# pacellie/raytracer_challenge

Measured on AMD Instinct MI355X. Metric: Mrays/s (unique rays: primary+shadow+reflection+refraction) at 1920x1080 depth-5, higher is better.
Workload: dtype f64

## Files before the change

### raytracer_challenge_amd/csrc/device_scene.h

```cpp
#pragma once
#include <stddef.h>
#include <stdint.h>

enum { OP_PRIM = 0, OP_GROUP = 1, OP_MESH = 2, OP_BVH = 3, OP_QUIRK = 4, OP_QGRID = 5, OP_CSG = 6, OP_CSG_END = 7 };

struct DOp {
  int32_t op, a, b, c;
  int32_t g;
  int32_t pad[3];
};

#define RTC_KOPS 12
#define RTC_KPLANES 6
struct DPlaneK {
  double row[4];
  int32_t prim;
  int32_t gcond;
  int32_t pad[2];
  double n[3];
};

struct DBvhNode {
  float lo0[3], hi0[3];
  float lo1[3], hi1[3];
// ... 165 lines not shown

struct DStats {
  unsigned long long rays_primary, rays_shadow, rays_reflect, rays_refract, rays_container;
  unsigned long long accel_nodes, group_tests, tri_tests, analytic_tests;
  unsigned long long knodes;
  unsigned long long kplanes;
  unsigned long long light_cells;
  unsigned long long kgroups;
  unsigned long long diag[64];
  unsigned long long nan_ts;
  unsigned long long guard;
  unsigned long long guard_claim;
  long long guard_info[8];
  unsigned long long wf_overflow;
};
#define RTC_STATS_LAUNCH_BYTES offsetof(DStats, nan_ts)

#define RTC_MAX_FUEL 16

#if defined(__HIPCC__) || defined(RTC_EMU)
#define RTC_HD __host__ __device__
#else
#define RTC_HD
#endif
static inline RTC_HD unsigned long long rtc_mix64(unsigned long long x) {
  x ^= x >> 33; x *= 0xff51afd7ed558ccdull; x ^= x >> 33; x *= 0xc4ceb9fe1a85ec53ull; x ^= x >> 33;
  return x;
}
static inline RTC_HD unsigned long long rtc_hit_hash_base(unsigned long long t_bits, int32_t prim, int32_t push) {
  return rtc_mix64(t_bits) ^ ((((unsigned long long)(uint32_t)prim << 32) | (unsigned long long)(uint32_t)push) * 0x9E3779B97F4A7C15ull);
}
static inline RTC_HD unsigned long long rtc_hit_hash(unsigned long long base, int depth, int kind) {
  return rtc_mix64(base ^ ((unsigned long long)(((unsigned)depth << 8) | (unsigned)kind) + 1ull) * 0xD6E8FEB86659FD93ull);
}

static inline RTC_HD unsigned long long rtc_splitmix64(unsigned long long z) {
  z = (z ^ (z >> 30)) * 0xbf58476d1ce4e5b9ull; z = (z ^ (z >> 27)) * 0x94d049bb133111ebull;
  return z ^ (z >> 31);
}
static inline RTC_HD unsigned long long rtc_area_hash(int light, double x, double y, double z) {
  unsigned long long bx, by, bz;
  __builtin_memcpy(&bx, &x, 8); __builtin_memcpy(&by, &y, 8); __builtin_memcpy(&bz, &z, 8);
  return rtc_splitmix64(rtc_splitmix64(rtc_splitmix64(rtc_splitmix64((unsigned long long)(uint32_t)light) ^ bx) ^ by) ^ bz);
}
static inline RTC_HD double rtc_area_jitter(unsigned long long h, unsigned j) {
  return (double)(rtc_splitmix64(h ^ (unsigned long long)j) >> 11) * 0x1.0p-53;
}
#define RTC_ALIGHT 16
#define RTC_SLIGHT 22

#define RTC_WF_SHADE_COUNT 32
#define RTC_WF_OVERFLOW 63
#define RTC_WF_CHUNK_NEXT 64
#define RTC_WF_COUNTS (64 + 32 * 8 * (RTC_MAX_FUEL + 2))
#ifndef RTC_WF_CHUNK
#define RTC_WF_CHUNK 64u
#endif
#define RTC_SR_PLAIN 0x40000000
#define RTC_WF_MISS (-2)
struct DWave {
  double* rq[2];
  double* h_t;
  int32_t* h_prim;
  double* h_n12;
  double* sr;
  int32_t* sr_mat;
  int32_t* sr_node;
  double* contrib;
  int32_t* child;
  uint32_t* counts;
  uint32_t cap;
  uint32_t pad;
  unsigned long long* dig;
};
static inline uint64_t dwave_bytes(uint64_t cap, int levels) {
  return cap * (uint64_t)(7 + 7 + 1 + 2 + 9 + 3 * levels) * sizeof(double) + (cap * (uint64_t)(1 + 1 + 1 + 2 * levels) + RTC_WF_COUNTS) * sizeof(int32_t);
}
static inline void dwave_carve(DWave* W, void* mem, uint64_t cap, int levels) {
  double* d = (double*)mem;
  W->rq[0] = d; d += 7 * cap;
  W->rq[1] = d; d += 7 * cap;
  W->h_t = d; d += cap;
  W->h_n12 = d; d += 2 * cap;
  W->sr = d; d += 9 * cap;
  W->contrib = d; d += 3 * (uint64_t)levels * cap;
  int32_t* q = (int32_t*)d;
  W->h_prim = q; q += cap;
  W->sr_mat = q; q += cap;
  W->sr_node = q; q += cap;
  W->child = q; q += 2 * (uint64_t)levels * cap;
  W->counts = (uint32_t*)q;
  W->cap = (uint32_t)cap;
  W->pad = 0;
  W->dig = nullptr;
}
#ifndef RTC_BVH_STACK
#define RTC_BVH_STACK 64
#endif
```

### raytracer_challenge_amd/csrc/rtc_background.hip

```cpp
#include "rtc_device.hpp"

#ifdef RTC_BG_BUILD

template <>
void rtc_launch_trace_bg_build<RTC_BG_BUILD>(const RtcFrame& F, const DBackground& bg, unsigned grid, int fuel, double* rgb) {
  constexpr RtcVariant R = RTC_BG_BUILDS[RTC_BG_BUILD];
  DSceneBg S;
  static_cast<DScene&>(S) = F.S;
  S.bg = bg;
  if (F.count)
    hipLaunchKernelGGL((rtc_trace_kernel<true, R.feat, R.kops, 0, false, R.area, R.uv, R.spot, true>), dim3(grid), dim3(RTC_BLOCK), rtc_stack_bytes(F.S), F.stream, S, F.cam, F.pm, fuel,
                       rgb, F.hit_t, F.hit_prim, F.hit_k, F.stats);
  else
    hipLaunchKernelGGL((rtc_trace_kernel<false, R.feat, R.kops, 0, false, R.area, R.uv, R.spot, true>), dim3(grid), dim3(RTC_BLOCK), rtc_stack_bytes(F.S), F.stream, S, F.cam, F.pm, fuel,
                       rgb, F.hit_t, F.hit_prim, F.hit_k, F.stats);
}

#else

uint64_t rtc_wavefront_work(const DCamera& cam, const DPixelMap& pm);

template <bool UV>
__global__ void __launch_bounds__(256) wf_background(DScene S, DCamera cam, DPixelMap pm, DWave W, int level, unsigned n0, DBackground bg) {
  const WorkMap wm = make_workmap(pm, cam);
  const unsigned count = wf_count(W, level, n0);
  const size_t cap = W.cap;
  int32_t* ch = W.child + (size_t)level * 2 * cap;
  double* cb = W.contrib + (size_t)level * 3 * cap;
  const double* rq = W.rq[level & 1];
  for (unsigned long long i = (unsigned long long)blockIdx.x * blockDim.x + threadIdx.x; i < count; i += (unsigned long long)gridDim.x * blockDim.x) {
    double dx, dy, dz, weight = 1.0;
    if (level == 0) {
      uint64_t q = 0;
      if (!work_to_slot(wm, i, q)) continue;
      if (ch[i] != RTC_WF_MISS) continue;
      const Ray r = slot_ray(pm, cam, q);
      dx = r.dx; dy = r.dy; dz = r.dz;
    } else {
      if (ch[i] != RTC_WF_MISS) continue;
      dx = rq[3 * cap + i]; dy = rq[4 * cap + i]; dz = rq[5 * cap + i];
      weight = rq[6 * cap + i];
    }
    double r, g, b;
    background_color<UV>(S, bg, dx, dy, dz, r, g, b);
    cb[i] = weight * r; cb[cap + i] = weight * g; cb[2 * cap + i] = weight * b;
    ch[i] = -1;
  }
}

void rtc_launch_wf_background(const DScene& S, const DCamera& cam, const DPixelMap& pm, const DWave& W, int level, unsigned n0, const DBackground& bg, unsigned blocks,
                              hipStream_t stream) {
  const unsigned long long most = level == 0 ? n0 : W.cap;
  const dim3 grid((unsigned)std::max<unsigned long long>(1ull, std::min<unsigned long long>((most + 255ull) / 256ull, (unsigned long long)std::max(1u, blocks)))), block(256);
  if (S.has_uv) hipLaunchKernelGGL(wf_background<true>, grid, block, 0, stream, S, cam, pm, W, level, n0, bg);
  else hipLaunchKernelGGL(wf_background<false>, grid, block, 0, stream, S, cam, pm, W, level, n0, bg);
}

template <bool UV>
__global__ void __launch_bounds__(256) rtc_background_colors_kernel(DScene S, DBackground bg, const double* __restrict__ dirs, unsigned long long n, double* __restrict__ rgb) {
  for (unsigned long long i = (unsigned long long)blockIdx.x * blockDim.x + threadIdx.x; i < n; i += (unsigned long long)gridDim.x * blockDim.x) {
    double r, g, b;
    background_color<UV>(S, bg, dirs[3 * i], dirs[3 * i + 1], dirs[3 * i + 2], r, g, b);
    rgb[3 * i] = r; rgb[3 * i + 1] = g; rgb[3 * i + 2] = b;
  }
}
void rtc_launch_background_colors(const DScene& S, const DBackground& bg, const double* dirs, unsigned long long n, double* rgb, hipStream_t stream) {
  if (n == 0) return;
  const dim3 grid((unsigned)std::min<unsigned long long>((n + 255ull) / 256ull, 8192ull)), block(256);
  if (S.has_uv) hipLaunchKernelGGL(rtc_background_colors_kernel<true>, grid, block, 0, stream, S, bg, dirs, n, rgb);
  else hipLaunchKernelGGL(rtc_background_colors_kernel<false>, grid, block, 0, stream, S, bg, dirs, n, rgb);
}

void rtc_launch_trace_bg(const DScene& S, const DBackground& bg, const DCamera& cam, const DPixelMap& pm, int fuel, double* rgb, double* hit_t, int* hit_prim, int* hit_k,
                         DStats* stats, bool count, hipStream_t stream) {
  if (pm.n == 0) return;
  const unsigned grid = (unsigned)((rtc_wavefront_work(cam, pm) + RTC_BLOCK - 1) / RTC_BLOCK);
  const RtcFrame F = {S, cam, pm, hit_t, hit_prim, hit_k, stats, stream, count};
  switch (rtc_pick_bg_build(S.has_area != 0, S.has_uv != 0, S.has_spot != 0)) {
    case 0: return rtc_launch_trace_bg_build<0>(F, bg, grid, fuel, rgb);
    case 1: return rtc_launch_trace_bg_build<1>(F, bg, grid, fuel, rgb);
    case 2: return rtc_launch_trace_bg_build<2>(F, bg, grid, fuel, rgb);
    case 3: return rtc_launch_trace_bg_build<3>(F, bg, grid, fuel, rgb);
    case 4: return rtc_launch_trace_bg_build<4>(F, bg, grid, fuel, rgb);
// ... 7 lines not shown
```

### raytracer_challenge_amd/csrc/rtc_device.hpp

```cpp
#pragma once

#include <hip/hip_runtime.h>
#include <stdint.h>

#include <algorithm>
#include <type_traits>

#include "background_point.h"
#include "device_scene.h"
#include "spot_factor.h"

#define EPS 0.00001
#ifndef RTC_BLOCK
#define RTC_BLOCK 64
#endif
#ifndef RTC_WAVES_PER_SIMD
#define RTC_WAVES_PER_SIMD 1
#endif
#ifdef RTC_TRAVERSE_NOINLINE
#define TRAVERSE_INLINE __noinline__
#else
#define TRAVERSE_INLINE __forceinline__
#endif
#ifndef RTC_LANE_ID
// ... 1484 lines not shown
            Pending& p = pend[np++];
            p.ox = st.ux; p.oy = st.uy; p.oz = st.uz; p.dx = spawn.tdx; p.dy = spawn.tdy; p.dz = spawn.tdz;
            p.weight = spawn.wt; p.fuel = fuel - 1; p.kind = 2;
          }
          if (spawn.refl) {
            ray.ox = st.px; ray.oy = st.py; ray.oz = st.pz; ray.dx = st.rx; ray.dy = st.ry; ray.dz = st.rz;
            weight = spawn.wr; fuel = fuel - 1; kind = 1;
            continue;
          }
          if (spawn.refr) {
            ray.ox = st.ux; ray.oy = st.uy; ray.oz = st.uz; ray.dx = spawn.tdx; ray.dy = spawn.tdy; ray.dz = spawn.tdz;
            weight = spawn.wt; fuel = fuel - 1; kind = 2;
            continue;
          }
        }
      } else if constexpr (BG) {
        double br, bgr, bb;
        background_color<UV>(S, S.bg, ray.dx, ray.dy, ray.dz, br, bgr, bb);
        acc_r += weight * br; acc_g += weight * bgr; acc_b += weight * bb;
      }
      DIAG_REGION(5);
      if (np == 0) {
        rgb[3 * q + 0] = acc_r;
        rgb[3 * q + 1] = acc_g;
        rgb[3 * q + 2] = acc_b;
        if (COUNT && pm.digest) pm.digest[q] = dg;
        break;
      }
      const Pending& p = pend[--np];
      ray.ox = p.ox; ray.oy = p.oy; ray.oz = p.oz; ray.dx = p.dx; ray.dy = p.dy; ray.dz = p.dz;
      weight = p.weight; fuel = p.fuel; kind = p.kind;
    }
  }

#ifdef RTC_DIAG
  atomicAdd(&s_diag[14], __builtin_amdgcn_s_memtime() - diag_k0);
  atomicAdd(&s_diag[15], 1ull);
  __syncthreads();
  if (threadIdx.x < 64 && s_diag[threadIdx.x]) atomicAdd(&stats->diag[threadIdx.x], s_diag[threadIdx.x]);
#endif
  if (C.nan_ts) atomicAdd(&stats->nan_ts, (unsigned long long)C.nan_ts);
  if (COUNT) {
    atomicAdd(&stats->rays_primary, (unsigned long long)n_primary);
    atomicAdd(&stats->rays_shadow, (unsigned long long)n_shadow);
    atomicAdd(&stats->rays_reflect, (unsigned long long)n_reflect);
    atomicAdd(&stats->rays_refract, (unsigned long long)n_refract);
    atomicAdd(&stats->rays_container, (unsigned long long)n_container);
    publish_counters(stats, C);
  }
}

namespace {

__device__ __forceinline__ unsigned wf_count(const DWave& W, int level, unsigned n0) {
  if (level == 0) return n0;
  unsigned c = W.counts[level];
  return c < W.cap ? c : W.cap;
}
__device__ __forceinline__ Ray wf_load_ray(const DWave& W, int level, unsigned i, double& weight) {
  const double* q = W.rq[level & 1];
  const size_t cap = W.cap;
  Ray r;
  r.ox = q[i]; r.oy = q[cap + i]; r.oz = q[2 * cap + i]; r.dx = q[3 * cap + i]; r.dy = q[4 * cap + i]; r.dz = q[5 * cap + i];
  weight = q[6 * cap + i];
  return r;
}

struct RecView {
  double ex, ey, ez, weight;
};
__device__ __forceinline__ RecView shade_rec_view(const DCamera& cam, const DPixelMap& pm, const DWave& W, const WorkMap& wm, int level, int node) {
  if (level == 0) {
    uint64_t q = 0;
    (void)work_to_slot(wm, (unsigned)node, q);
    const Ray pr = slot_ray(pm, cam, q);
    return {-pr.dx, -pr.dy, -pr.dz, 1.0};
  }
  const double* rq = W.rq[level & 1];
  const size_t cap = W.cap;
  return {-rq[3 * cap + node], -rq[4 * cap + node], -rq[5 * cap + node], rq[6 * cap + node]};
}
__device__ __forceinline__ const double* shade_rec_material(const DScene& S, const DWave& W, unsigned s, double& cr, double& cg, double& cb) {
  const double* r = W.sr;
  const size_t cap = W.cap;
  const int mrow = W.sr_mat[s];
  const double* M = S.mat + 8 * (mrow & (RTC_SR_PLAIN - 1));
  if (mrow & RTC_SR_PLAIN) { cr = M[4]; cg = M[5]; cb = M[6]; }
  else { cr = r[6 * cap + s]; cg = r[7 * cap + s]; cb = r[8 * cap + s]; }
  return M;
}
__device__ __forceinline__ const double* shade_rec_material_row(const DScene& S, const DWave& W, unsigned s, int mrow, double& cr, double& cg, double& cb) {
  const double* r = W.sr;
  const size_t cap = W.cap;
  const double* M = S.mat + 8 * (mrow & (RTC_SR_PLAIN - 1));
  if (mrow & RTC_SR_PLAIN) { cr = M[4]; cg = M[5]; cb = M[6]; }
  else { cr = r[6 * cap + s]; cg = r[7 * cap + s]; cb = r[8 * cap + s]; }
  return M;
}

}

template <int FEAT, bool KOPS, bool LDSC>
__device__ __forceinline__ void wf_trace_ray(const DScene& S, const DCamera& cam, const DPixelMap& pm, const DWave& W, const WorkMap& wm, int level, unsigned i,
                                             double* __restrict__ hit_t, int* __restrict__ hit_prim, int* __restrict__ hit_k, int* stack, int stride, Counters& C,
                                             unsigned& n_rays, unsigned& n_container, int fuel_left, const LdsScene& L, bool digest = false) {
  const size_t cap = W.cap;
  int32_t* ch = W.child + (size_t)level * 2 * cap;
  Ray ray;
  uint64_t q = 0;
  if (level == 0) {
    if (!work_to_slot(wm, i, q)) { W.h_prim[i] = -1; return; }
// ... 87 lines not shown
    if (RTC_PROBE & 8) RTC_LAUNDER(qx);
    const ShadowRay sh = shadow_ray(qx, py, pz, LG[3], LG[4], LG[5]);
    phong_add(LG, sh.ray.dx, sh.ray.dy, sh.ray.dz, (shadow_mask >> li) & 1ull, nx, ny, nz, v.ex, v.ey, v.ez, cr, cg, cbl, M[0], M[1], M[2], M[3], sr, sg, sb);
  }
  cb[node] = v.weight * sr; cb[cap + node] = v.weight * sg; cb[2 * cap + node] = v.weight * sb;
  DIAG_SPAN_END(5);
}

template <int FEAT, bool KOPS, bool LDSC, bool SPOT = false>
__device__ __forceinline__ void wf_shadow_rec_area(const DScene& S, const DCamera& cam, const DPixelMap& pm, const DWave& W, const WorkMap& wm, int level, unsigned s,
                                                   int* stack, int stride, Counters& C, unsigned& n_shadow, const LdsScene& L) {
  const size_t cap = W.cap;
  double* cb = W.contrib + (size_t)level * 3 * cap;
  const double* r = W.sr;
  const int node = W.sr_node[s];
  const RecView v = shade_rec_view(cam, pm, W, wm, level, node);
  double cr, cg, cbl;
  const double* M = shade_rec_material(S, W, s, cr, cg, cbl);
  double sr = 0.0, sg = 0.0, sb = 0.0;
  shade_lights_area<FEAT, KOPS, LDSC, false, SPOT>(S, r[s], r[cap + s], r[2 * cap + s], r[3 * cap + s], r[4 * cap + s], r[5 * cap + s], v.ex, v.ey, v.ez, cr, cg, cbl, M[0], M[1],
                                             M[2], M[3], C, stack, stride, n_shadow, L, sr, sg, sb);
  cb[node] = v.weight * sr; cb[cap + node] = v.weight * sg; cb[2 * cap + node] = v.weight * sb;
}

#ifndef RTC_WF_TS_WAVES
#define RTC_WF_TS_WAVES 3
#endif
#ifndef RTC_WF_TS_WAVES_MAXFEAT
#define RTC_WF_TS_WAVES_MAXFEAT 1
#endif
#ifndef RTC_LDS_BLOCK
#define RTC_LDS_BLOCK (256 * RTC_WF_TS_WAVES)
#endif
template <bool COUNT, int FEAT, bool KOPS, bool LDSC = false, bool AREA = false, bool SPOT = false>
__global__ void __launch_bounds__(LDSC ? RTC_LDS_BLOCK : RTC_BLOCK, (KOPS || FEAT <= RTC_WF_TS_WAVES_MAXFEAT) ? RTC_WF_TS_WAVES : 2) wf_ts(DScene S, DCamera cam, DPixelMap pm, DWave W, int tl, int sl, unsigned n0, int slot, int fuel_left,
                                                                     double* __restrict__ hit_t, int* __restrict__ hit_prim, int* __restrict__ hit_k, DStats* __restrict__ stats) {
  RTC_LDS_STACK(lds_stack);
  LdsScene L = {nullptr, nullptr, nullptr, nullptr, 0, 0, 0};
  int* stack = lds_stack + threadIdx.x;
  int stride = RTC_BLOCK;
#ifndef RTC_EMU
  if (LDSC) {
    stack = (int*)lds_fill(S, (char*)lds_stack, L) + threadIdx.x;
    stride = (int)blockDim.x;
  }
#endif
  Counters C = {0, 0, 0, 0, 0, 0, 0, 0, 0};
  unsigned n_rays = 0, n_container = 0, n_shadow = 0;
#ifdef RTC_DIAG
  if (threadIdx.x < 64) s_diag[threadIdx.x] = 0ull;
  __syncthreads();
#endif
  const WorkMap wm = make_workmap(pm, cam);
  const unsigned nt = tl >= 0 ? wf_count(W, tl, n0) : 0u;
  unsigned ns = sl >= 0 ? W.counts[RTC_WF_SHADE_COUNT + sl] : 0u;
  if (ns > W.cap) ns = W.cap;
  const unsigned ct = (nt + RTC_WF_CHUNK - 1) / RTC_WF_CHUNK, cs = (ns + RTC_WF_CHUNK - 1) / RTC_WF_CHUNK;
  const unsigned nx = gridDim.x < 8u ? gridDim.x : 8u;
  const unsigned x = blockIdx.x % nx;
  unsigned* next = &W.counts[RTC_WF_CHUNK_NEXT + 32 * (8 * slot + (int)x)];
  const int lane = RTC_LANE_ID;
  for (;;) {
    unsigned kx = 0;
    if (lane == 0) kx = atomicAdd(next, 1u);
    kx = __shfl(kx, 0);
    const unsigned long long chunk = (unsigned long long)kx * nx + x;
    if (chunk >= (unsigned long long)ct + cs) break;
    if (chunk < ct) {
      const unsigned base = (unsigned)chunk * RTC_WF_CHUNK;
      for (unsigned o = 0; o < RTC_WF_CHUNK; o += RTC_WF_LANES) {
        const unsigned i = base + o + (unsigned)lane;
        if (i < nt) {
          DIAG_SPAN_BEGIN();
          wf_trace_ray<FEAT, KOPS, LDSC>(S, cam, pm, W, wm, tl, i, hit_t, hit_prim, hit_k, stack, stride, C, n_rays, n_container, fuel_left, L, COUNT && W.dig != nullptr);
          DIAG_SPAN_END(7);
        }
      }
    } else {
      const unsigned base = (unsigned)(chunk - ct) * RTC_WF_CHUNK;
      for (unsigned o = 0; o < RTC_WF_CHUNK; o += RTC_WF_LANES) {
        const unsigned s = base + o + (unsigned)lane;
        if (s < ns) {
          DIAG_SPAN_BEGIN();
          if constexpr (AREA) wf_shadow_rec_area<FEAT, KOPS, LDSC, SPOT>(S, cam, pm, W, wm, sl, s, stack, stride, C, n_shadow, L);
          else wf_shadow_rec<FEAT, KOPS, LDSC, KOPS && !COUNT && FEAT <= RTC_WF_TS_WAVES_MAXFEAT>(S, cam, pm, W, wm, sl, s, stack, stride, C, n_shadow, L);
          DIAG_SPAN_END(7);
        }
      }
    }
  }
  if (C.nan_ts) atomicAdd(&stats->nan_ts, (unsigned long long)C.nan_ts);
#ifdef RTC_DIAG
  __syncthreads();
  if (threadIdx.x < 64 && s_diag[threadIdx.x]) atomicAdd(&stats->diag[threadIdx.x], s_diag[threadIdx.x]);
#endif
  if (COUNT) {
    if (tl == 0) atomicAdd(&stats->rays_primary, (unsigned long long)n_rays);
    atomicAdd(&stats->rays_container, (unsigned long long)n_container);
    atomicAdd(&stats->rays_shadow, (unsigned long long)n_shadow);
    publish_counters(stats, C);
  }
}

struct RtcVariant {
  int feat;
  bool kops;
  bool area;
  bool uv;
  bool spot;
};
constexpr RtcVariant RTC_VARIANTS[] = {
    {0, true, false, false, false},
    {1, true, false, false, false},
    {1, false, false, false, false},
    {2, false, false, false, false},
    {3, false, false, false, false},
    {2, true, false, false, false},
    {3, false, true, false, false},
    {1, true, true, false, false},
    {3, false, false, true, false},
    {3, false, true, true, false},
    {3, false, true, false, true},
    {3, false, true, true, true},
};
constexpr int RTC_N_VARIANTS = (int)(sizeof(RTC_VARIANTS) / sizeof(RTC_VARIANTS[0]));
constexpr bool rtc_v_wavefront(RtcVariant r) { return !r.uv; }
constexpr bool rtc_v_lds(RtcVariant r) { return r.kops && !r.area && !r.uv; }
constexpr bool rtc_v_trace_3wave(RtcVariant r) { return r.feat == 1 && !r.area && !r.uv; }
constexpr bool rtc_v_trace_lean(RtcVariant r) { return r.feat <= 1 && !r.area && !r.uv; }

constexpr int rtc_pick_variant(int feat, bool kops, bool area, bool uv, bool spot, bool wavefront) {
  if (spot) return (uv && !wavefront) ? 11 : 10;
  if (uv && !wavefront) return area ? 9 : 8;
  if (area) return (feat <= 1 && kops) ? 7 : 6;
  if (feat <= 1 && kops) return feat;
  if (feat == 2 && kops) return 5;
  return feat <= 1 ? 2 : feat + 1;
}

enum RtcTraceBuild { RTC_TB_DEFAULT = 0, RTC_TB_COUNT = 1, RTC_TB_LEAN = 2, RTC_TB_3WAVE = 3 };
enum RtcWfTsBuild { RTC_TS_MEM = 0, RTC_TS_MEM_COUNT = 1, RTC_TS_LDS = 2, RTC_TS_LDS_COUNT = 3 };
enum RtcWfShadeBuild { RTC_SH_COUNT = 0, RTC_SH_COUNT_UV = 1, RTC_SH_UV = 2, RTC_SH_PIPE_LV0 = 3, RTC_SH_PIPE = 4, RTC_SH_PAT = 5 };
// ... 85 lines not shown
```

### raytracer_challenge_amd/csrc/rtc_kernels.hip

```cpp
#include <cstdio>
#include <cstdlib>
#include <utility>

#include "../../include/rtc.h"
#include "rtc_device.hpp"

#ifdef RTC_EMU
#include "rtc_feat.hip"
constexpr int RTC_VARIANTS_BUILT = 6;
#else
constexpr int RTC_VARIANTS_BUILT = RTC_N_VARIANTS;
#endif
template <int... V>
static const RtcVariantOps& rtc_ops(int v, std::integer_sequence<int, V...>) {
  static const RtcVariantOps ops[RTC_N_VARIANTS] = {rtc_variant_ops<V>()...};
  return ops[v];
}
static const RtcVariantOps& rtc_ops(int v) { return rtc_ops(v, std::make_integer_sequence<int, RTC_VARIANTS_BUILT>{}); }
static int rtc_variant(const DScene& S, bool wavefront) {
  return rtc_pick_variant(rtc_scene_feat(S), S.n_kops > 0, S.has_area != 0, S.has_uv != 0, S.has_spot != 0, wavefront);
}

#ifndef RTC_WF_SHADE_WAVES
#define RTC_WF_SHADE_WAVES 4
#endif
namespace {
struct WfShadeIn {
  int prim;
  Ray ray;
  double weight, t;
};
__device__ __forceinline__ int wf_shade_fetch_prim(const DWave& W, unsigned long long i, unsigned count) { return i < count ? W.h_prim[i] : -1; }
template <bool LV0>
__device__ __forceinline__ WfShadeIn wf_shade_prefetch(const DWave& W, int level, unsigned long long i, int lane, unsigned count, int prim) {
  const unsigned long long first = i - (unsigned)lane;
  const unsigned j = prim >= 0 ? (unsigned)i : (first < count ? (unsigned)first : 0u);
  WfShadeIn in = {prim, {0.0, 0.0, 0.0, 0.0, 0.0, 0.0}, 1.0, 0.0};
  if (!LV0) in.ray = wf_load_ray(W, level, j, in.weight);
  in.t = W.h_t[j];
  return in;
}
#ifndef RTC_EMU
__device__ __forceinline__ unsigned wf_row_scan16(unsigned v) {
  v += (unsigned)__builtin_amdgcn_update_dpp(0, (int)v, 0x111, 0xf, 0xf, true);
  v += (unsigned)__builtin_amdgcn_update_dpp(0, (int)v, 0x112, 0xf, 0xf, true);
  v += (unsigned)__builtin_amdgcn_update_dpp(0, (int)v, 0x114, 0xf, 0xf, true);
  v += (unsigned)__builtin_amdgcn_update_dpp(0, (int)v, 0x118, 0xf, 0xf, true);
  return v;
}
#endif
}
template <bool COUNT, bool PAT = true, bool UV = false, bool PIPE = false, bool LV0 = false, bool NP = false>
__global__ void __launch_bounds__(RTC_WF_SHADE_BLOCK, RTC_WF_SHADE_WAVES) wf_shade(std::conditional_t<NP, DSceneNp, DScene> S, DCamera cam, DPixelMap pm, DWave W, int level, unsigned n0, int fuel0, DStats* __restrict__ stats) {
  constexpr int n_waves = RTC_WF_SHADE_BLOCK >= 64 ? RTC_WF_SHADE_BLOCK / 64 : 1;
  static_assert(n_waves <= 8, "wf_shade: eight counters per class");
  __shared__ unsigned s_cnt2[2][40];
  unsigned parity = 0;
  const WorkMap wm = make_workmap(pm, cam);
  const unsigned count = wf_count(W, level, n0);
  const size_t cap = W.cap;
  const double L = (double)S.n_lights;
  const int fuel = fuel0 - level;
  unsigned n_reflect = 0, n_refract = 0;
  int32_t* ch = W.child + (size_t)level * 2 * cap;
  double* nq = W.rq[(level + 1) & 1];
  const int lane = RTC_LANE_ID;
  const int wave = (int)(threadIdx.x / (RTC_WF_SHADE_BLOCK >= 64 ? 64 : 1));
  const unsigned long long step = (unsigned long long)gridDim.x * RTC_WF_SHADE_BLOCK;
  WfShadeIn nx = {-1, {0.0, 0.0, 0.0, 0.0, 0.0, 0.0}, 1.0, 0.0};
  int nx_prim = -1;
  const bool level0 = PIPE ? LV0 : level == 0;
  if (PIPE) {
    const unsigned long long i0 = (unsigned long long)blockIdx.x * RTC_WF_SHADE_BLOCK + threadIdx.x;
    nx = wf_shade_prefetch<LV0>(W, level, i0, lane, count, wf_shade_fetch_prim(W, i0, count));
  }
  for (unsigned long long base = (unsigned long long)blockIdx.x * RTC_WF_SHADE_BLOCK; base < count; base += step) {
    const unsigned i = (unsigned)base + threadIdx.x;
    const WfShadeIn in = nx;
    const int prim = PIPE ? in.prim : wf_shade_fetch_prim(W, i, count);
    if (PIPE) nx_prim = wf_shade_fetch_prim(W, base + step + threadIdx.x, count);
    const bool hit = prim >= 0;
    State st;
    double cr = 0.0, cg = 0.0, cbl = 0.0, weight = 1.0, n1 = 1.0, n2 = 1.0;
    int mat = 0, shading_row = 0, geom = 0;
    double reflective = 0.0, transparency = 0.0;
    if (hit) {
      Ray ray;
      if (level0) {
        uint64_t q = 0;
        (void)work_to_slot(wm, i, q);
        ray = slot_ray(pm, cam, q);
      } else if (PIPE) {
        ray = in.ray;
        weight = in.weight;
      } else {
        ray = wf_load_ray(W, level, i, weight);
      }
      const DPrim P = S.prims[prim];
      geom = P.geom;
      const double* M = S.mat + 8 * P.mat;
      reflective = M[4]; transparency = M[5];
      mat = ~P.mat;
      if (PIPE) shading_row = (int)M[7];
      double hu, hv;
      hit_uv(S, P, ray, hu, hv);
      if constexpr (NP) prepare_state<true>(S, P, ray, W.h_t[i], hu, hv, st, &S.bump);
      else prepare_state(S, P, ray, PIPE ? in.t : W.h_t[i], hu, hv, st);
      if (transparency != 0.0 && fuel > 0) { n1 = W.h_n12[i]; n2 = W.h_n12[cap + i]; }
      if constexpr (PAT) {
        if (S.pats[S.mat_pattern[P.mat]].tag != 1) {
          pattern_at<UV>(S, P, st, cr, cg, cbl);
          mat = P.mat;
        }
      }
    }
    const bool blend = hit && reflective > 0.0 && transparency > 0.0;
    double R = 0.0;
    if (blend) {
      R = blend_reflectance(st, n1, n2, fuel, cr, cg, cbl);
      if (R != R && mat < 0) mat = ~mat;
    }
    ChildRays spawn = {false, false, 0.0, 0.0, 0.0, 0.0, 0.0};
    if (hit && fuel > 0) spawn = child_rays(st, n1, n2, weight, L, reflective, transparency, blend, R);
    const unsigned long long lt = (1ull << lane) - 1ull;
    const bool on_plane = hit && geom == 1;
    const unsigned long long m_rec0 = __ballot(hit && on_plane ? 1 : 0), m_rec1 = __ballot(hit && !on_plane ? 1 : 0);
    const unsigned long long m_c0 = __ballot(spawn.refl && on_plane ? 1 : 0), m_c1 = __ballot(spawn.refl && !on_plane ? 1 : 0), m_c2 = __ballot(spawn.refr ? 1 : 0);
    unsigned* s_cnt = s_cnt2[parity];
    parity ^= 1u;
    if (lane == 0) {
      s_cnt[wave] = (unsigned)__popcll(m_rec0); s_cnt[8 + wave] = (unsigned)__popcll(m_rec1);
      s_cnt[16 + wave] = (unsigned)__popcll(m_c0); s_cnt[24 + wave] = (unsigned)__popcll(m_c1); s_cnt[32 + wave] = (unsigned)__popcll(m_c2);
    }
    if (PIPE) nx = wf_shade_prefetch<LV0>(W, level, base + step + threadIdx.x, lane, count, nx_prim);
    __syncthreads();
#ifndef RTC_EMU
    if (PIPE && n_waves == 8 && wave == 0) {
      const unsigned c = lane < 40 ? s_cnt[lane] : 0u;
      const unsigned in_row = wf_row_scan16(c);
      const unsigned tr = (unsigned)__builtin_amdgcn_readlane((int)in_row, 15), t1 = (unsigned)__builtin_amdgcn_readlane((int)in_row, 31);
      const unsigned tc = t1 + (unsigned)__builtin_amdgcn_readlane((int)in_row, 39);
      const unsigned total = lane == 0 ? tr : tc;
      unsigned old = 0u;
      if (lane < 2 && total) {
        old = atomicAdd(&W.counts[lane == 0 ? RTC_WF_SHADE_COUNT + level : level + 1], total);
        if ((unsigned long long)old + total > W.cap) { W.counts[RTC_WF_OVERFLOW] = 1u; stats->wf_overflow = 1ull; }
      }
      const unsigned br = (unsigned)__builtin_amdgcn_readlane((int)old, 0), bc = (unsigned)__builtin_amdgcn_readlane((int)old, 1);
      if (lane < 40) s_cnt[lane] = (lane < 16 ? br : bc + (lane >= 32 ? t1 : 0u)) + in_row - c;
    }
    if (!PIPE || n_waves != 8)
#endif
    if (threadIdx.x == 0) {
      unsigned tr = 0, tc = 0;
      for (int w = 0; w < n_waves; w++) { tr += s_cnt[w] + s_cnt[8 + w]; tc += s_cnt[16 + w] + s_cnt[24 + w] + s_cnt[32 + w]; }
      unsigned br = tr ? atomicAdd(&W.counts[RTC_WF_SHADE_COUNT + level], tr) : 0u;
      unsigned bc = tc ? atomicAdd(&W.counts[level + 1], tc) : 0u;
      if ((unsigned long long)br + tr > W.cap || (unsigned long long)bc + tc > W.cap) { W.counts[RTC_WF_OVERFLOW] = 1u; stats->wf_overflow = 1ull; }
      for (int k = 0; k < 2; k++)
        for (int w = 0; w < n_waves; w++) { unsigned r = s_cnt[8 * k + w]; s_cnt[8 * k + w] = br; br += r; }
      for (int k = 2; k < 5; k++)
        for (int w = 0; w < n_waves; w++) { unsigned c = s_cnt[8 * k + w]; s_cnt[8 * k + w] = bc; bc += c; }
    }
    __syncthreads();
    const unsigned s = on_plane ? s_cnt[wave] + (unsigned)__popcll(m_rec0 & lt) : s_cnt[8 + wave] + (unsigned)__popcll(m_rec1 & lt);
    const unsigned jr = on_plane ? s_cnt[16 + wave] + (unsigned)__popcll(m_c0 & lt) : s_cnt[24 + wave] + (unsigned)__popcll(m_c1 & lt);
    const unsigned jt = s_cnt[32 + wave] + (unsigned)__popcll(m_c2 & lt);
    if (hit && s < W.cap) {
      double* r = W.sr;
      r[s] = st.px; r[cap + s] = st.py; r[2 * cap + s] = st.pz;
      r[3 * cap + s] = st.nx; r[4 * cap + s] = st.ny; r[5 * cap + s] = st.nz;
      if (mat >= 0) {
        r[6 * cap + s] = cr; r[7 * cap + s] = cg; r[8 * cap + s] = cbl;
        W.sr_mat[s] = mat;
      } else {
        if (!PIPE) shading_row = (int)S.mat[8 * ~mat + 7];
        W.sr_mat[s] = RTC_SR_PLAIN | shading_row;
      }
      W.sr_node[s] = (int32_t)i;
    }
    if (spawn.refl && jr < W.cap) {
      nq[jr] = st.px; nq[cap + jr] = st.py; nq[2 * cap + jr] = st.pz; nq[3 * cap + jr] = st.rx; nq[4 * cap + jr] = st.ry; nq[5 * cap + jr] = st.rz;
      nq[6 * cap + jr] = spawn.wr;
      ch[i] = (int32_t)jr;
      n_reflect++;
    }
    if (spawn.refr && jt < W.cap) {
      nq[jt] = st.ux; nq[cap + jt] = st.uy; nq[2 * cap + jt] = st.uz; nq[3 * cap + jt] = spawn.tdx; nq[4 * cap + jt] = spawn.tdy; nq[5 * cap + jt] = spawn.tdz;
      nq[6 * cap + jt] = spawn.wt;
      ch[cap + i] = (int32_t)jt;
      n_refract++;
    }
  }
  if (COUNT) {
    atomicAdd(&stats->rays_reflect, (unsigned long long)n_reflect);
    atomicAdd(&stats->rays_refract, (unsigned long long)n_refract);
  }
}

__global__ void __launch_bounds__(256) wf_gather(DCamera cam, DPixelMap pm, DWave W, unsigned n0, double* __restrict__ rgb) {
  const WorkMap wm = make_workmap(pm, cam);
  const size_t cap = W.cap;
  for (unsigned i = blockIdx.x * blockDim.x + threadIdx.x; i < n0; i += gridDim.x * blockDim.x) {
    uint64_t q;
    if (!work_to_slot(wm, i, q)) continue;
    double r = 0.0, g = 0.0, b = 0.0;
    int wait_idx[RTC_MAX_FUEL + 1];
    int wait_lvl[RTC_MAX_FUEL + 1];
    int sp = 0, lvl = 0, idx = (int)i;
    const bool digest = W.dig != nullptr && pm.digest != nullptr;
    unsigned long long dg = 0ull;
    int kind = 0;
    for (;;) {
      const double* cb = W.contrib + (size_t)lvl * 3 * cap;
      const int32_t* ch = W.child + (size_t)lvl * 2 * cap;
// ... 181 lines not shown
```

### raytracer_challenge_amd/csrc/rtc_scene.cpp

```cpp
#include <hip/hip_runtime_api.h>

#include <algorithm>
#include <atomic>
#include <chrono>
#include <cmath>
#include <condition_variable>
#include <cstdlib>
#include <cstdio>
#include <cstring>
#include <deque>
#include <functional>
#include <initializer_list>
#include <memory>
#include <mutex>
#include <string>
#include <thread>
#include <vector>

#include "../../include/rtc.h"
#include "adaptive_contrast.h"
#include "background_point.h"
#include "bump_normal.h"
#include "camera_sampling.h"
#include "device_scene.h"
// ... 285 lines not shown
  if (tuned) path = pick_path(s, launch_signature(cam, pm, fuel), rtc_wavefront_work(cam, pm), fuel, will_sync, pm.mode != 2);
  if (path == 4 && s->wave_alloc_failed && force == 0) path = 1;
  const bool wavefront = path == 4 && pm.n > 0;
  if (s->d.csg_max_hits > RTC_CSG_MAX_HITS) {
    const uint64_t threads = wavefront ? (uint64_t)s->wave_blocks * 64ull : ((rtc_wavefront_work(cam, pm) + 63) / 64) * 64;
    if (threads > s->csg_slab_threads) {
      const uint64_t bytes = threads * (uint64_t)s->d.csg_max_hits * sizeof(DCsgHit);
      const char* e = std::getenv("RTC_CSG_MAX_BYTES");
      if (bytes > (e ? std::strtoull(e, nullptr, 10) : (16ull << 30)))
        return rtc_fail(RTC_ERR_UNSUPPORTED, "the CSG intersection slab of this launch exceeds RTC_CSG_MAX_BYTES: render fewer pixels per call");
      const int rc = grow(&s->csg_slab_threads, threads, {{(void**)&s->csg_slab, bytes}}, s->stream);
      if (rc != RTC_OK) return rc;
    }
    s->d.csg_slab = s->csg_slab;
  }
  if (wavefront) {
    int rc = ensure_wave(s, rtc_wavefront_work(cam, pm), fuel);
    if (rc == RTC_ERR_UNSUPPORTED && force == 0) {
      if (tuned) drop_wavefront(s);
      else s->wave_alloc_failed = true;
      return run(s, cam, pm, fuel, d_rgb, want_hits, stats, count, sync, 1, after);
    }
    if (rc != RTC_OK) return rc;
    s->wave.dig = nullptr;
    if (pm.digest && count) {
      const uint64_t need = (uint64_t)s->wave_cap * (uint64_t)(fuel + 1);
      rc = grow(&s->cap_wave_dig, need, {{(void**)&s->d_wave_dig, need * sizeof(unsigned long long)}}, s->stream);
      if (rc != RTC_OK) return rc;
      s->wave.dig = s->d_wave_dig;
    }
    HIP_OK(hipMemsetAsync(s->wave.counts, 0, RTC_WF_COUNTS * sizeof(uint32_t), s->stream));
    HIP_OK(hipEventRecord(s->ev0, s->stream));
    rtc_launch_wavefront(s->d, cam, pm, fuel, s->wave, d_rgb, want_hits ? s->d_hit_t : nullptr, s->d_hit_prim, s->d_hit_k, s->d_stats, count, s->stream, s->wave_blocks, s->shade_blocks, s->lds_bytes,
                         s->has_bg ? &s->bg : nullptr, s->has_bump ? &s->bump : nullptr);
  } else if (s->has_bump) {
    rtc_launch_trace_np(s->d, s->bump, s->has_bg ? &s->bg : nullptr, cam, pm, fuel, d_rgb, want_hits ? s->d_hit_t : nullptr, s->d_hit_prim, s->d_hit_k, s->d_stats, count, s->stream);
  } else if (s->has_bg) {
    rtc_launch_trace_bg(s->d, s->bg, cam, pm, fuel, d_rgb, want_hits ? s->d_hit_t : nullptr, s->d_hit_prim, s->d_hit_k, s->d_stats, count, s->stream);
  } else {
    rtc_launch_trace(s->d, cam, pm, fuel, d_rgb, want_hits ? s->d_hit_t : nullptr, s->d_hit_prim, s->d_hit_k, s->d_stats, count, s->stream, rtc_scene_is_big(s->bytes));
  }
  HIP_OK(hipGetLastError());
  HIP_OK(hipEventRecord(s->ev1, s->stream));
  s->last_wavefront = wavefront;
  s->last_fuel = fuel;
  if (after) { int rca = (*after)(); if (rca != RTC_OK) return rca; }
  if (!sync && !stats) return RTC_OK;
  HIP_OK(hipStreamSynchronize(s->stream));
  DStats h;
  int rcs = read_clear_sticky(s, &h);
  if (rcs != RTC_OK) return rcs;
  if (wavefront) {
    if (std::getenv("RTC_WF_DUMP_COUNTS")) {
      uint32_t c[64];
      HIP_OK(hipMemcpy(c, s->wave.counts, sizeof(c), hipMemcpyDeviceToHost));
      std::fprintf(stderr, "[rtc-wf] level: rays / shade records:");
      for (int l = 0; l <= fuel; l++) std::fprintf(stderr, " %d: %u / %u;", l, l ? c[l] : (unsigned)rtc_wavefront_work(cam, pm), c[RTC_WF_SHADE_COUNT + l]);
      std::fprintf(stderr, "\n");
    }
    uint32_t overflow = 0;
    HIP_OK(hipMemcpy(&overflow, s->wave.counts + RTC_WF_OVERFLOW, sizeof(overflow), hipMemcpyDeviceToHost));
    if (overflow) {
      const uint64_t n_work = rtc_wavefront_work(cam, pm);
      if (s->wave_eighths < 512 && wave_bytes(wave_cap(n_work, 2 * s->wave_eighths), fuel + 1) <= wave_budget() && wave_cap(n_work, 2 * s->wave_eighths) <= 0x7fffff00ull) {
        s->wave_eighths *= 2;
        const int rc2 = run(s, cam, pm, fuel, d_rgb, want_hits, stats, count, true, 4, after);
        if (rc2 != RTC_ERR_UNSUPPORTED) return rc2;
      }
      if (tuned) drop_wavefront(s);
      return run(s, cam, pm, fuel, d_rgb, want_hits, stats, count, true, 1, after);
    }
  }
  if (tuned && !count && pm.mode == 2 && !s->tune_choice) {
    float ms = 0.f;
    HIP_OK(hipEventElapsedTime(&ms, s->ev0, s->ev1));
    record_sample(s, wavefront, ms);
  }
  if (stats) {
    int rcf = fill_stats(s, h, pm.n, stats);
    if (rcf != RTC_OK) return rcf;
  }
  if (std::getenv("RTC_DIAG_DUMP")) {
    std::fprintf(stderr, "[rtc-diag]");
    for (int i = 0; i < 64; i++) std::fprintf(stderr, " %llu", (unsigned long long)h.diag[i]);
    std::fprintf(stderr, "\n");
  }
  if (h.guard) return rtc_fail(RTC_ERR_DEVICE, "traversal guard tripped (mask " + std::to_string(h.guard) + "): an index left its array; no pixel since the last check is trustworthy");
  if (h.nan_ts) return rtc_fail(RTC_ERR_NAN, "a NaN intersection t reached a sort of two or more intersections (the reference panics in Intersection::sort, src/intersection.rs:124)");
  return RTC_OK;
}

int make_pixel_map(rtc_scene* s, uint64_t hsize, uint64_t total, const uint64_t* pixel_indices, uint64_t first, uint64_t n, DPixelMap* pm, std::vector<uint64_t>* range_idx) {
  *pm = DPixelMap{};
  pm->n = n;
  if (!pixel_indices) {
    if (first % hsize == 0 && n % hsize == 0) {
      pm->mode = 2; pm->row_first = (uint32_t)(first / hsize); pm->row_step = 1;
    } else {
      range_idx->resize(n);
      for (uint64_t i = 0; i < n; i++) (*range_idx)[i] = first + i;
      pixel_indices = range_idx->data();
    }
  }
  if (pixel_indices) {
    for (uint64_t i = 0; i < n; i++)
      if (pixel_indices[i] >= total) return rtc_fail(RTC_ERR_INVALID, "pixel index exceeds the image");
    const int rc = grow(&s->cap_idx, n, {{(void**)&s->d_idx, n * sizeof(uint64_t)}});
    if (rc != RTC_OK) return rc;
    HIP_OK(hipMemcpy(s->d_idx, pixel_indices, n * sizeof(uint64_t), hipMemcpyHostToDevice));
    pm->mode = 1; pm->indices = s->d_idx;
// ... 1684 lines not shown
```

Baseline: 12900.

## Split wavefront queues into near/far halves filled from both ends

Wavefront ray and shadow-record queues are now filled from both ends: plane/near records grow from the bottom and the rest from the top, with separate counters for each. The trace kernel walks four segments (rays top/bottom, shadow records top/bottom) as separate chunk ranges, so rays of similar kind sit together and wave divergence should drop. Overflow detection is reworked to check the combined counts. This adds index remapping and extra atomics per block, and more bookkeeping in the chunk scheduler.

```diff
diff --git a/raytracer_challenge_amd/csrc/device_scene.h b/raytracer_challenge_amd/csrc/device_scene.h
--- a/raytracer_challenge_amd/csrc/device_scene.h
+++ b/raytracer_challenge_amd/csrc/device_scene.h
@@ -241,7 +241,9 @@
 #define RTC_WF_SHADE_COUNT 32
 #define RTC_WF_OVERFLOW 63
 #define RTC_WF_CHUNK_NEXT 64
-#define RTC_WF_COUNTS (64 + 32 * 8 * (RTC_MAX_FUEL + 2))
+#define RTC_WF_TOP_COUNT (64 + 32 * 8 * (RTC_MAX_FUEL + 2))
+#define RTC_WF_SHADE_TOP_COUNT (RTC_WF_TOP_COUNT + 32)
+#define RTC_WF_COUNTS (RTC_WF_TOP_COUNT + 64)
 #ifndef RTC_WF_CHUNK
 #define RTC_WF_CHUNK 64u
 #endif
diff --git a/raytracer_challenge_amd/csrc/rtc_background.hip b/raytracer_challenge_amd/csrc/rtc_background.hip
--- a/raytracer_challenge_amd/csrc/rtc_background.hip
+++ b/raytracer_challenge_amd/csrc/rtc_background.hip
@@ -23,12 +23,14 @@
 template <bool UV>
 __global__ void __launch_bounds__(256) wf_background(DScene S, DCamera cam, DPixelMap pm, DWave W, int level, unsigned n0, DBackground bg) {
   const WorkMap wm = make_workmap(pm, cam);
-  const unsigned count = wf_count(W, level, n0);
+  const WfParts parts = wf_count(W, level, n0);
+  const unsigned count = parts.top + parts.bottom;
   const size_t cap = W.cap;
   int32_t* ch = W.child + (size_t)level * 2 * cap;
   double* cb = W.contrib + (size_t)level * 3 * cap;
   const double* rq = W.rq[level & 1];
-  for (unsigned long long i = (unsigned long long)blockIdx.x * blockDim.x + threadIdx.x; i < count; i += (unsigned long long)gridDim.x * blockDim.x) {
+  for (unsigned long long w = (unsigned long long)blockIdx.x * blockDim.x + threadIdx.x; w < count; w += (unsigned long long)gridDim.x * blockDim.x) {
+    const unsigned i = wf_index(parts, W.cap, (unsigned)w);
     double dx, dy, dz, weight = 1.0;
     if (level == 0) {
       uint64_t q = 0;
diff --git a/raytracer_challenge_amd/csrc/rtc_device.hpp b/raytracer_challenge_amd/csrc/rtc_device.hpp
--- a/raytracer_challenge_amd/csrc/rtc_device.hpp
+++ b/raytracer_challenge_amd/csrc/rtc_device.hpp
@@ -1560,11 +1560,23 @@
 
 namespace {
 
-__device__ __forceinline__ unsigned wf_count(const DWave& W, int level, unsigned n0) {
-  if (level == 0) return n0;
-  unsigned c = W.counts[level];
-  return c < W.cap ? c : W.cap;
-}
+struct WfParts {
+  unsigned top, bottom;
+};
+__device__ __forceinline__ WfParts wf_parts(const DWave& W, unsigned top, unsigned bottom) {
+  WfParts p;
+  p.top = top < W.cap ? top : W.cap;
+  p.bottom = bottom < W.cap - p.top ? bottom : W.cap - p.top;
+  return p;
+}
+__device__ __forceinline__ WfParts wf_count(const DWave& W, int level, unsigned n0) {
+  if (level == 0) return {0u, n0};
+  return wf_parts(W, W.counts[RTC_WF_TOP_COUNT + level], W.counts[level]);
+}
+__device__ __forceinline__ WfParts wf_rec_count(const DWave& W, int level) {
+  return wf_parts(W, W.counts[RTC_WF_SHADE_TOP_COUNT + level], W.counts[RTC_WF_SHADE_COUNT + level]);
+}
+__device__ __forceinline__ unsigned wf_index(const WfParts& p, unsigned cap, unsigned w) { return w < p.top ? cap - p.top + w : w - p.top; }
 __device__ __forceinline__ Ray wf_load_ray(const DWave& W, int level, unsigned i, double& weight) {
   const double* q = W.rq[level & 1];
   const size_t cap = W.cap;
@@ -1758,10 +1770,9 @@
   __syncthreads();
 #endif
   const WorkMap wm = make_workmap(pm, cam);
-  const unsigned nt = tl >= 0 ? wf_count(W, tl, n0) : 0u;
-  unsigned ns = sl >= 0 ? W.counts[RTC_WF_SHADE_COUNT + sl] : 0u;
-  if (ns > W.cap) ns = W.cap;
-  const unsigned ct = (nt + RTC_WF_CHUNK - 1) / RTC_WF_CHUNK, cs = (ns + RTC_WF_CHUNK - 1) / RTC_WF_CHUNK;
+  const WfParts pt = tl >= 0 ? wf_count(W, tl, n0) : WfParts{0u, 0u};
+  const WfParts ps = sl >= 0 ? wf_rec_count(W, sl) : WfParts{0u, 0u};
+  const unsigned n_a = pt.top, n_b = pt.bottom, n_c = ps.top, n_d = ps.bottom;
   const unsigned nx = gridDim.x < 8u ? gridDim.x : 8u;
   const unsigned x = blockIdx.x % nx;
   unsigned* next = &W.counts[RTC_WF_CHUNK_NEXT + 32 * (8 * slot + (int)x)];
@@ -1771,22 +1782,29 @@
     if (lane == 0) kx = atomicAdd(next, 1u);
     kx = __shfl(kx, 0);
     const unsigned long long chunk = (unsigned long long)kx * nx + x;
-    if (chunk >= (unsigned long long)ct + cs) break;
-    if (chunk < ct) {
-      const unsigned base = (unsigned)chunk * RTC_WF_CHUNK;
+    if (chunk >= 0x80000000ull) break;
+    unsigned c = (unsigned)chunk, part_n = n_a;
+    int part = 0;
+    for (; part < 3 && c >= (part_n + RTC_WF_CHUNK - 1) / RTC_WF_CHUNK; part++) {
+      c -= (part_n + RTC_WF_CHUNK - 1) / RTC_WF_CHUNK;
+      part_n = part == 0 ? n_b : part == 1 ? n_c : n_d;
+    }
+    if (c >= (part_n + RTC_WF_CHUNK - 1) / RTC_WF_CHUNK) break;
+    const unsigned origin = (part & 1) == 0 ? W.cap - part_n : 0u;
+    const unsigned base = c * RTC_WF_CHUNK;
+    if (part < 2) {
       for (unsigned o = 0; o < RTC_WF_CHUNK; o += RTC_WF_LANES) {
-        const unsigned i = base + o + (unsigned)lane;
-        if (i < nt) {
+        const unsigned i = origin + base + o + (unsigned)lane;
+        if (base + o + (unsigned)lane < part_n) {
           DIAG_SPAN_BEGIN();
           wf_trace_ray<FEAT, KOPS, LDSC>(S, cam, pm, W, wm, tl, i, hit_t, hit_prim, hit_k, stack, stride, C, n_rays, n_container, fuel_left, L, COUNT && W.dig != nullptr);
           DIAG_SPAN_END(7);
         }
       }
     } else {
-      const unsigned base = (unsigned)(chunk - ct) * RTC_WF_CHUNK;
       for (unsigned o = 0; o < RTC_WF_CHUNK; o += RTC_WF_LANES) {
-        const unsigned s = base + o + (unsigned)lane;
-        if (s < ns) {
+        const unsigned s = origin + base + o + (unsigned)lane;
+        if (base + o + (unsigned)lane < part_n) {
           DIAG_SPAN_BEGIN();
           if constexpr (AREA) wf_shadow_rec_area<FEAT, KOPS, LDSC, SPOT>(S, cam, pm, W, wm, sl, s, stack, stride, C, n_shadow, L);
           else wf_shadow_rec<FEAT, KOPS, LDSC, KOPS && !COUNT && FEAT <= RTC_WF_TS_WAVES_MAXFEAT>(S, cam, pm, W, wm, sl, s, stack, stride, C, n_shadow, L);
@@ -1794,6 +1812,10 @@
         }
       }
     }
+  }
+  if ((tl > 0 && (unsigned long long)W.counts[RTC_WF_TOP_COUNT + tl] + W.counts[tl] > W.cap) ||
+      (sl >= 0 && (unsigned long long)W.counts[RTC_WF_SHADE_TOP_COUNT + sl] + W.counts[RTC_WF_SHADE_COUNT + sl] > W.cap)) {
+    if (blockIdx.x == 0 && threadIdx.x == 0) { W.counts[RTC_WF_OVERFLOW] = 1u; stats->wf_overflow = 1ull; }
   }
   if (C.nan_ts) atomicAdd(&stats->nan_ts, (unsigned long long)C.nan_ts);
 #ifdef RTC_DIAG
diff --git a/raytracer_challenge_amd/csrc/rtc_kernels.hip b/raytracer_challenge_amd/csrc/rtc_kernels.hip
--- a/raytracer_challenge_amd/csrc/rtc_kernels.hip
+++ b/raytracer_challenge_amd/csrc/rtc_kernels.hip
@@ -30,11 +30,13 @@
   Ray ray;
   double weight, t;
 };
-__device__ __forceinline__ int wf_shade_fetch_prim(const DWave& W, unsigned long long i, unsigned count) { return i < count ? W.h_prim[i] : -1; }
+__device__ __forceinline__ int wf_shade_fetch_prim(const DWave& W, const WfParts& parts, unsigned long long w, unsigned count) {
+  return w < count ? W.h_prim[wf_index(parts, W.cap, (unsigned)w)] : -1;
+}
 template <bool LV0>
-__device__ __forceinline__ WfShadeIn wf_shade_prefetch(const DWave& W, int level, unsigned long long i, int lane, unsigned count, int prim) {
-  const unsigned long long first = i - (unsigned)lane;
-  const unsigned j = prim >= 0 ? (unsigned)i : (first < count ? (unsigned)first : 0u);
+__device__ __forceinline__ WfShadeIn wf_shade_prefetch(const DWave& W, const WfParts& parts, int level, unsigned long long w, int lane, unsigned count, int prim) {
+  const unsigned long long first = w - (unsigned)lane;
+  const unsigned j = prim >= 0 ? wf_index(parts, W.cap, (unsigned)w) : (first < count ? wf_index(parts, W.cap, (unsigned)first) : 0u);
   WfShadeIn in = {prim, {0.0, 0.0, 0.0, 0.0, 0.0, 0.0}, 1.0, 0.0};
   if (!LV0) in.ray = wf_load_ray(W, level, j, in.weight);
   in.t = W.h_t[j];
@@ -52,12 +54,15 @@
 }
 template <bool COUNT, bool PAT = true, bool UV = false, bool PIPE = false, bool LV0 = false, bool NP = false>
 __global__ void __launch_bounds__(RTC_WF_SHADE_BLOCK, RTC_WF_SHADE_WAVES) wf_shade(std::conditional_t<NP, DSceneNp, DScene> S, DCamera cam, DPixelMap pm, DWave W, int level, unsigned n0, int fuel0, DStats* __restrict__ stats) {
+  constexpr int end_of[5] = {0, 1, 2, 3, 3};
   constexpr int n_waves = RTC_WF_SHADE_BLOCK >= 64 ? RTC_WF_SHADE_BLOCK / 64 : 1;
   static_assert(n_waves <= 8, "wf_shade: eight counters per class");
   __shared__ unsigned s_cnt2[2][40];
   unsigned parity = 0;
   const WorkMap wm = make_workmap(pm, cam);
-  const unsigned count = wf_count(W, level, n0);
+  const bool level0 = PIPE ? LV0 : level == 0;
+  const WfParts parts = level0 ? WfParts{0u, n0} : wf_count(W, level, n0);
+  const unsigned count = parts.top + parts.bottom;
   const size_t cap = W.cap;
   const double L = (double)S.n_lights;
   const int fuel = fuel0 - level;
@@ -69,16 +74,15 @@
   const unsigned long long step = (unsigned long long)gridDim.x * RTC_WF_SHADE_BLOCK;
   WfShadeIn nx = {-1, {0.0, 0.0, 0.0, 0.0, 0.0, 0.0}, 1.0, 0.0};
   int nx_prim = -1;
-  const bool level0 = PIPE ? LV0 : level == 0;
   if (PIPE) {
-    const unsigned long long i0 = (unsigned long long)blockIdx.x * RTC_WF_SHADE_BLOCK + threadIdx.x;
-    nx = wf_shade_prefetch<LV0>(W, level, i0, lane, count, wf_shade_fetch_prim(W, i0, count));
+    const unsigned long long w0 = (unsigned long long)blockIdx.x * RTC_WF_SHADE_BLOCK + threadIdx.x;
+    nx = wf_shade_prefetch<LV0>(W, parts, level, w0, lane, count, wf_shade_fetch_prim(W, parts, w0, count));
   }
   for (unsigned long long base = (unsigned long long)blockIdx.x * RTC_WF_SHADE_BLOCK; base < count; base += step) {
-    const unsigned i = (unsigned)base + threadIdx.x;
+    const unsigned i = wf_index(parts, W.cap, (unsigned)base + threadIdx.x);
     const WfShadeIn in = nx;
-    const int prim = PIPE ? in.prim : wf_shade_fetch_prim(W, i, count);
-    if (PIPE) nx_prim = wf_shade_fetch_prim(W, base + step + threadIdx.x, count);
+    const int prim = PIPE ? in.prim : wf_shade_fetch_prim(W, parts, base + threadIdx.x, count);
+    if (PIPE) nx_prim = wf_shade_fetch_prim(W, parts, base + step + threadIdx.x, count);
     const bool hit = prim >= 0;
     State st;
     double cr = 0.0, cg = 0.0, cbl = 0.0, weight = 1.0, n1 = 1.0, n2 = 1.0;
@@ -132,35 +136,47 @@
       s_cnt[wave] = (unsigned)__popcll(m_rec0); s_cnt[8 + wave] = (unsigned)__popcll(m_rec1);
       s_cnt[16 + wave] = (unsigned)__popcll(m_c0); s_cnt[24 + wave] = (unsigned)__popcll(m_c1); s_cnt[32 + wave] = (unsigned)__popcll(m_c2);
     }
-    if (PIPE) nx = wf_shade_prefetch<LV0>(W, level, base + step + threadIdx.x, lane, count, nx_prim);
+    if (PIPE) nx = wf_shade_prefetch<LV0>(W, parts, level, base + step + threadIdx.x, lane, count, nx_prim);
     __syncthreads();
 #ifndef RTC_EMU
     if (PIPE && n_waves == 8 && wave == 0) {
       const unsigned c = lane < 40 ? s_cnt[lane] : 0u;
       const unsigned in_row = wf_row_scan16(c);
-      const unsigned tr = (unsigned)__builtin_amdgcn_readlane((int)in_row, 15), t1 = (unsigned)__builtin_amdgcn_readlane((int)in_row, 31);
-      const unsigned tc = t1 + (unsigned)__builtin_amdgcn_readlane((int)in_row, 39);
-      const unsigned total = lane == 0 ? tr : tc;
-      unsigned old = 0u;
-      if (lane < 2 && total) {
-        old = atomicAdd(&W.counts[lane == 0 ? RTC_WF_SHADE_COUNT + level : level + 1], total);
-        if ((unsigned long long)old + total > W.cap) { W.counts[RTC_WF_OVERFLOW] = 1u; stats->wf_overflow = 1ull; }
-      }
-      const unsigned br = (unsigned)__builtin_amdgcn_readlane((int)old, 0), bc = (unsigned)__builtin_amdgcn_readlane((int)old, 1);
-      if (lane < 40) s_cnt[lane] = (lane < 16 ? br : bc + (lane >= 32 ? t1 : 0u)) + in_row - c;
+      const unsigned r0 = (unsigned)__builtin_amdgcn_readlane((int)in_row, 7), r01 = (unsigned)__builtin_amdgcn_readlane((int)in_row, 15);
+      const unsigned k0 = (unsigned)__builtin_amdgcn_readlane((int)in_row, 23), k01 = (unsigned)__builtin_amdgcn_readlane((int)in_row, 31);
+      const unsigned k2 = (unsigned)__builtin_amdgcn_readlane((int)in_row, 39);
+      const unsigned t_rn = r0, t_rf = r01 - r0, t_cn = k0, t_cf = k01 - k0 + k2;
+      const unsigned total = lane == 0 ? t_rn : lane == 1 ? t_rf : lane == 2 ? t_cn : t_cf;
+      unsigned first = 0u;
+      if (lane < 4 && total) {
+        const int row = lane == 0 ? RTC_WF_SHADE_COUNT + level : lane == 1 ? RTC_WF_SHADE_TOP_COUNT + level : lane == 2 ? level + 1 : RTC_WF_TOP_COUNT + level + 1;
+        const unsigned old = atomicAdd(&W.counts[row], total);
+        const bool fits = (unsigned long long)old + total <= W.cap;
+        if (!fits) { W.counts[RTC_WF_OVERFLOW] = 1u; stats->wf_overflow = 1ull; }
+        first = (lane & 1) ? (fits ? W.cap - old - total : W.cap) : old;
+      }
+      const unsigned b_rn = (unsigned)__builtin_amdgcn_readlane((int)first, 0), b_rf = (unsigned)__builtin_amdgcn_readlane((int)first, 1);
+      const unsigned b_cn = (unsigned)__builtin_amdgcn_readlane((int)first, 2), b_cf = (unsigned)__builtin_amdgcn_readlane((int)first, 3);
+      if (lane < 40) {
+        const unsigned ex = in_row - c;
+        s_cnt[lane] = lane < 8 ? b_rn + ex : lane < 16 ? b_rf + ex - r0 : lane < 24 ? b_cn + ex : lane < 32 ? b_cf + ex - k0 : b_cf + k01 - k0 + ex;
+      }
     }
     if (!PIPE || n_waves != 8)
 #endif
     if (threadIdx.x == 0) {
-      unsigned tr = 0, tc = 0;
-      for (int w = 0; w < n_waves; w++) { tr += s_cnt[w] + s_cnt[8 + w]; tc += s_cnt[16 + w] + s_cnt[24 + w] + s_cnt[32 + w]; }
-      unsigned br = tr ? atomicAdd(&W.counts[RTC_WF_SHADE_COUNT + level], tr) : 0u;
-      unsigned bc = tc ? atomicAdd(&W.counts[level + 1], tc) : 0u;
-      if ((unsigned long long)br + tr > W.cap || (unsigned long long)bc + tc > W.cap) { W.counts[RTC_WF_OVERFLOW] = 1u; stats->wf_overflow = 1ull; }
-      for (int k = 0; k < 2; k++)
-        for (int w = 0; w < n_waves; w++) { unsigned r = s_cnt[8 * k + w]; s_cnt[8 * k + w] = br; br += r; }
-      for (int k = 2; k < 5; k++)
-        for (int w = 0; w < n_waves; w++) { unsigned c = s_cnt[8 * k + w]; s_cnt[8 * k + w] = bc; bc += c; }
+      unsigned t[4] = {0u, 0u, 0u, 0u}, b[4];
+      for (int k = 0; k < 5; k++)
+        for (int w = 0; w < n_waves; w++) t[end_of[k]] += s_cnt[8 * k + w];
+      const int row[4] = {RTC_WF_SHADE_COUNT + level, RTC_WF_SHADE_TOP_COUNT + level, level + 1, RTC_WF_TOP_COUNT + level + 1};
+      for (int e = 0; e < 4; e++) {
+        const unsigned old = t[e] ? atomicAdd(&W.counts[row[e]], t[e]) : 0u;
+        const bool fits = (unsigned long long)old + t[e] <= W.cap;
+        if (!fits) { W.counts[RTC_WF_OVERFLOW] = 1u; stats->wf_overflow = 1ull; }
+        b[e] = (e & 1) ? (fits ? W.cap - old - t[e] : W.cap) : old;
+      }
+      for (int k = 0; k < 5; k++)
+        for (int w = 0; w < n_waves; w++) { const unsigned r = s_cnt[8 * k + w]; s_cnt[8 * k + w] = b[end_of[k]]; b[end_of[k]] += r; }
     }
     __syncthreads();
     const unsigned s = on_plane ? s_cnt[wave] + (unsigned)__popcll(m_rec0 & lt) : s_cnt[8 + wave] + (unsigned)__popcll(m_rec1 & lt);
diff --git a/raytracer_challenge_amd/csrc/rtc_scene.cpp b/raytracer_challenge_amd/csrc/rtc_scene.cpp
--- a/raytracer_challenge_amd/csrc/rtc_scene.cpp
+++ b/raytracer_challenge_amd/csrc/rtc_scene.cpp
@@ -361,10 +361,12 @@
   if (rcs != RTC_OK) return rcs;
   if (wavefront) {
     if (std::getenv("RTC_WF_DUMP_COUNTS")) {
-      uint32_t c[64];
+      uint32_t c[64], top[64];
       HIP_OK(hipMemcpy(c, s->wave.counts, sizeof(c), hipMemcpyDeviceToHost));
-      std::fprintf(stderr, "[rtc-wf] level: rays / shade records:");
-      for (int l = 0; l <= fuel; l++) std::fprintf(stderr, " %d: %u / %u;", l, l ? c[l] : (unsigned)rtc_wavefront_work(cam, pm), c[RTC_WF_SHADE_COUNT + l]);
+      HIP_OK(hipMemcpy(top, s->wave.counts + RTC_WF_TOP_COUNT, sizeof(top), hipMemcpyDeviceToHost));
+      std::fprintf(stderr, "[rtc-wf] level: rays far + near / shade records far + near:");
+      for (int l = 0; l <= fuel; l++)
+        std::fprintf(stderr, " %d: %u + %u / %u + %u;", l, top[l], l ? c[l] : (unsigned)rtc_wavefront_work(cam, pm), top[32 + l], c[RTC_WF_SHADE_COUNT + l]);
       std::fprintf(stderr, "\n");
     }
     uint32_t overflow = 0;
```

After: 13080, median of 6. 1.4% higher.
